# robin-karlsson0/pc-accumulation-lib

Measured on AMD Instinct MI355X. Metric: Mpoints/s projected+accumulated and BEV frames/s @256x256; 1/2/4/8 GPU, higher is better.
Workload: dtype f64; 1 GPU; KITTI-360 single forward cam, 120k pts/frame, 200 m horizon (~201 live frames, 5169634 stored pts), one 256x256x21 BEV per integrated frame; points_per_frame=120000, bev_px=256, view_m=80

## Files before the change

include/pca.h:

```cpp
#ifndef PCA_H
#define PCA_H

#include <stdint.h>

#ifdef __cplusplus
extern "C" {
#endif

#define PCA_VERSION 2

typedef struct pca_ctx pca_ctx;

typedef struct {
    double *x, *y, *z;
    float *intensity;
    uint32_t *rgbs;
    int32_t *inst;
    uint8_t *dyn;
    int64_t capacity;
    uint32_t *frame_box;
} pca_store;

#define PCA_STATUS_STORE_OVERFLOW 1u
#define PCA_STATUS_UV_OUT_OF_IMAGE 2u
// ... 121 lines not shown
    double *planes;
    uint16_t *planes_f16;
} pca_bev_job;
int pca_bev_generate_many(pca_ctx *ctx, const pca_store *store, const double *intensity64 ,
                          const int64_t *frame_off , const pca_bev_job *jobs, int n_jobs, int64_t max_points,
                          void *workspace , int64_t workspace_bytes, void *stream);

int pca_image_to_nchw_f32(pca_ctx *ctx, const uint8_t *rgb , int H, int W, const float mean[3], const float std[3],
                          float *out , void *stream);

int pca_bev_warp(pca_ctx *ctx, const uint16_t *planes_f16 , uint16_t *out_f16 , int n_planes, int px,
                 double a_1, double a_2, double b_1, double b_2, void *stream);

int pca_host_ego_to_grid(const double *full, int F, const double R[9], double dx, double dy, double view, int px,
                         double *rows, int32_t *start);

typedef struct pca_host_track pca_host_track;
typedef struct {
    const void *pts;
    const void *rgb;
    const void *sem;
    const void *sem_gt;
    int32_t n;
    uint32_t host_mask;
} pca_kitti_obs;
int pca_kitti_integrate(pca_ctx *ctx, const pca_kitti_obs *obs, const double P[12], int H, int W,
                        const uint64_t filter_mask[4], const pca_store *store, int64_t *frame_off , int slot,
                        int sample_mode, pca_host_track *track, const double *T_new_prev, double horizon, int64_t *evicted,
                        double *path_length, void *stream);
void pca_host_camera_cone(const double P[12], int H, int W, double cone[15]);
int pca_host_view_hull(int F, const double *then , const float *box , const double *cone ,
                       const double now[12], const pca_bev_params *prm, int *first, int *last);
int pca_bev_bin_range(pca_ctx *ctx, int slot_first, int slot_last_plus1);
int pca_bev_view_hint(pca_ctx *ctx, int slot0, int F, const double *then, const float *box, const double *cone, const double now[12],
                      const pca_bev_params *prm);
void pca_f32_box_decode(const uint32_t *rows , int n, float *box );

int pca_k1_defer(pca_ctx *ctx, int on);
int pca_k1_flush(pca_ctx *ctx);
int pca_kitti_generate_bev(pca_ctx *ctx, const pca_store *store, const int64_t *frame_off , int slot_begin,
                           int slot_split, int slot_end, int64_t max_points, const pca_bev_params *prm,
                           const double *pending_Ts, const int *pending_slot_ends, int n_pending, int write_back,
                           void *workspace , int64_t workspace_bytes, uint16_t *planes_f16 ,
                           void *host_planes , const pca_host_track *track, double *traj_rows,
                           int32_t *traj_start, int32_t *n_rows, void *stream);

typedef struct {
    const pca_kitti_obs *obs; const double *P; int32_t H, W; const uint64_t *filter_mask; const pca_store *store;
    int64_t *frame_off; int32_t slot, sample_mode; pca_host_track *track; const double *T_new_prev; double horizon;
    int64_t evicted; double path_length; void *stream;
} pca_kitti_integrate_args;
int pca_kitti_integrate_v(pca_ctx *ctx, pca_kitti_integrate_args *a);
typedef struct {
    const pca_store *store; const int64_t *frame_off; int32_t slot_begin, slot_split, slot_end, pad0; int64_t max_points;
    const pca_bev_params *prm; const double *pending_Ts; const int *pending_slot_ends; int32_t n_pending, write_back;
    void *workspace; int64_t workspace_bytes; uint16_t *planes_f16; void *host_planes; const pca_host_track *track;
    double *traj_rows; int32_t *traj_start; int32_t n_rows, pad1; void *stream;
    int32_t hint_slot0, hint_F; const double *hint_then; const float *hint_box; const double *hint_cone; const double *hint_now;
    int32_t hinted, pad2;
} pca_kitti_generate_bev_args;
int pca_kitti_generate_bev_v(pca_ctx *ctx, pca_kitti_generate_bev_args *a);

int pca_host_stage_h2d(int n, const void *const *src, void *const *pinned, void *const *dev, const int64_t *bytes,
                       void *stream);

int pca_host_d2h_async(pca_ctx *ctx, const void *dev, void *pinned, int64_t bytes, void *stream);
// ... 35 lines not shown
```

pc-accumulation-lib_amd/csrc/pca_bev.hip:

```cpp
#include "pca_bev_common.h"
#include "pca_k1_body.h"
#include <cstdlib>
#include <mutex>

#define KEY_INVALID 0xffffffffu
#define TS 8
#define TCELLS (TS * TS)
#define NFK (2 * TCELLS)
#ifndef AB_THREADS
#define AB_THREADS 1024
#endif
#define MAX_G 512
#ifndef BIN_RUNR
#define BIN_RUNR 4
#endif
#ifndef BIN_WPE
#define BIN_WPE 4
#endif
#ifndef BIN_UNR
#define BIN_UNR 4
#endif
#ifndef BIN_REG_P
#define BIN_REG_P 12
#endif
// ... 1365 lines not shown
            s_dyn[threadIdx.x] = w;
        }
        for (int t = threadIdx.x; t < n_hist; t += AB_THREADS) s_h[t] = 0;
        __syncthreads();
        const ViewConst vc = view_const(a);
        const uint32_t set = a.k1_slot >= a.slot_split ? 1u : 0u;
        const int lane = threadIdx.x & 63;
        uint32_t rkey[PPT];
#pragma unroll
        for (int r = 0; r < PPT; ++r) {
            const bool kept = (km[r] >> lane) & 1ull;
            rkey[r] = view_key_lean(vc, (double)p[r].x, (double)p[r].y, (double)p[r].z, kept, set);
            if (rkey[r] != KEY_INVALID) atomicAdd(&s_h[rkey[r] >> hs], 1u);
        }
        __syncthreads();
        bin_scan_tables(a, s_h, s_cur, s_wsum, split, (int)blockIdx.x);
        __syncthreads();
        const uint32_t seg = (uint32_t)blockIdx.x * K1_SEG;
#pragma unroll
        for (int r = 0; r < PPT; ++r) {
            if (rkey[r] == KEY_INVALID) continue;
            const uint32_t pos = seg + atomicAdd(&s_cur[rkey[r] >> hs], 1u);
            bin_store<false>(a, s_dyn, pos, rkey[r], packed[r], (double)p[r].z, 0.0, p[r].w);
        }
    }
};
static_assert(K1_SEG == 1024 * 4, "a K1 piece holds one 1024 x 4 tile");
__global__ __launch_bounds__(AB_THREADS) __attribute__((amdgpu_waves_per_eu(BIN_WPE, BIN_WPE))) void bev_tile_bin_k1(const BevArgs a, const K1Args k)
{
    if ((int)blockIdx.x < a.Gk) k1_body<AB_THREADS, 4, false, false, false>(k, BinK1Tail{a});
    else bev_tile_bin_body<false>(a);
}

template <bool I64>
__global__ __launch_bounds__(AB_THREADS) __attribute__((amdgpu_waves_per_eu(BIN_WPE, BIN_WPE))) void bev_tile_bin(const BevArgs a) { bev_tile_bin_body<I64>(a); }
#if C_THREADS == 512
#define C_OCC __attribute__((amdgpu_waves_per_eu(6, 6)))
#else
#define C_OCC
#endif
template <bool I64>
__global__ __launch_bounds__(C_THREADS) C_OCC void bev_tile_cells(const BevArgs a) { bev_tile_cells_body<I64>(a); }
template <bool I64, bool EXTRA, bool OWN>
__global__ __launch_bounds__(H_THREADS) void bev_tile_cells_heavy(const BevArgs a) { bev_tile_cells_heavy_body<I64, EXTRA, OWN>(a); }
#define PCA_BEV_MANY_MAX 48
__constant__ BevArgs g_bev_many[PCA_BEV_MANY_MAX];
template <bool I64>
__global__ __launch_bounds__(AB_THREADS) __attribute__((amdgpu_waves_per_eu(BIN_WPE, BIN_WPE))) void bev_tile_bin_many()
{
    const BevArgs &a = g_bev_many[blockIdx.y];
    if ((int)blockIdx.x < a.G) bev_tile_bin_body<I64>(a);
}
template <bool I64>
__global__ __launch_bounds__(C_THREADS) C_OCC void bev_tile_cells_many()
{
    bev_tile_cells_body<I64>(g_bev_many[blockIdx.y]);
}
template <bool I64>
__global__ __launch_bounds__(H_THREADS) void bev_tile_cells_heavy_many()
{
    bev_tile_cells_heavy_body<I64, false, false>(g_bev_many[blockIdx.y]);
}
template <bool I64>
__global__ __launch_bounds__(AB_THREADS) __attribute__((amdgpu_waves_per_eu(BIN_WPE, BIN_WPE))) void bev_tile_bin_band(const BevArgs a) { bev_tile_bin_body<I64, true>(a); }
template <bool I64>
__global__ __launch_bounds__(C_THREADS) C_OCC void bev_tile_cells_band(const BevArgs a) { bev_tile_cells_body<I64, true>(a); }
// ... 210 lines not shown
}

static size_t bev_decide_split(BevArgs &a, bool tuned)
{
    const int sp = tuned ? (int)PCA_ENV_ONCE("PCA_BEV_SPLIT", 1) : 0;
    a.split = (sp && a.heavy_launched && !a.intensity64 && (size_t)a.T * 16 <= 128 * 1024) ? (sp == 2 ? 2 : 1) : 0;
    return (size_t)a.T * 8 * (a.split ? 2 : 1);
}

static int bev_decide_k1_ride(pca_ctx *ctx, const BevArgs &a, bool tuned, size_t lds, hipStream_t s, K1Args *k1a, int *nt)
{
    *nt = 0;
    if (!ctx->k1_pend.valid) return 0;
    if (!tuned) return pca_k1_flush_pending(ctx);
    const int fk = (int)PCA_ENV_ONCE("PCA_FUSE_K1", 1);
    const pca_ctx::K1Pending &pd = ctx->k1_pend;
    bool owed_ok = true;
    for (int k = 0; k < a.n_pend; ++k) owed_ok = owed_ok && a.pend_slot_end[k] <= pd.slot;
    const bool fuse = fk && owed_ok && !a.intensity64 && pd.stream == s && pd.slot == a.slot_end - 1 && pd.slot >= a.slot_begin &&
                      pd.frame_off == a.frame_off && pd.store.x == a.st.x && lds <= K1_RIDE_LDS && pd.fr.n <= K1_RIDE * K1_SEG &&
                      pd.fr.n <= a.max_points && pca_k1_prepare_pending(ctx, k1a, nt, s) == 0 && *nt <= K1_RIDE;
    if (PCA_ENV_ONCE("PCA_FUSE_DBG", 0) && !fuse)
        fprintf(stderr, "bev: K1 of slot %d not taken along: switch %d owed_ok %d i64 %d stream %d slot %d (window %d..%d) frame_off %d store %d lds %zu n %d max_points %lld nt %d\n",
                pd.slot, fk, (int)owed_ok, a.intensity64 != nullptr, pd.stream == s, pd.slot == a.slot_end - 1, a.slot_begin, a.slot_end,
                pd.frame_off == a.frame_off, pd.store.x == a.st.x, lds, pd.fr.n, (long long)a.max_points, *nt);
    if (fuse) return 0;
    *nt = 0;
    return pca_k1_flush_pending(ctx);
}

struct BevBinRange { bool given; int first, end; };
static int bev_decide_bin_range(pca_ctx *ctx, BevArgs &a, bool tuned, const BevBinRange &r)
{
    if (!r.given || !PCA_ENV_ONCE("PCA_BEV_CULL", 1) || (a.n_pend > 0 && a.write_back)) return 0;
    const int f = r.first > a.slot_begin ? r.first : a.slot_begin, e = r.end < a.slot_end ? r.end : a.slot_end;
    a.bin_first = f; a.bin_end = e < f ? f : e;
    if (!tuned) return 0;
    const int64_t pts = PCA_ENV_ONCE("PCA_BEV_ONE_ROUND_PTS", 14500);
    a.span_hint = ctx->heavy_hint_dev + 1;
    a.span_hint_known = ctx->heavy_hint[1];
    return (pts > 0 && a.span_hint_known != 0 && (int64_t)a.span_hint_known * 1024 <= pts * ctx->n_cu && a.G > ctx->n_cu) ? ctx->n_cu : 0;
}

static void bev_size_level1(pca_ctx *ctx, BevArgs &a, int nt, int one_round)
{
    if (nt == 0) { if (one_round > 0) { a.G = one_round; bev_table_order(a); } return; }
    const pca_ctx::K1Pending &pd = ctx->k1_pend;
    const int cap = max_groups(), G0 = a.G;
    if (one_round) one_round -= nt;
    a.G = one_round > 0 ? one_round + nt : (G0 + nt <= cap || (cap - 2 * nt) * 4 < 3 * G0) ? G0 + nt : cap - nt;
    a.Gk = nt; bev_table_order(a); a.k1_slot = pd.slot; a.k1_n = pd.fr.n;
    a.max_points = a.max_points - pd.fr.n;
}

static int bev_launch_raster(pca_ctx *ctx, const BevKernelSet &ks, const BevArgs &a, const K1Args *k1, size_t lds, hipStream_t s)
{
    if (k1) {
        PCA_LAUNCH_SHM(ctx, PCA_K_BEV_BIN, bev_tile_bin_k1, dim3(a.G), dim3(AB_THREADS), lds, s, a, *k1);
        pca_k1_pending_launched(ctx, s);
    } else PCA_LAUNCH_SHM(ctx, PCA_K_BEV_BIN, ks.bin, dim3(a.G), dim3(AB_THREADS), lds, s, a);
    PCA_LAUNCH(ctx, PCA_K_BEV_CELLS, ks.cells, dim3(a.T), dim3(C_THREADS), s, a);
    if (!a.heavy_launched) return 0;
    const int heavy_grid = a.T < ctx->n_cu ? a.T : ctx->n_cu;
    const BevKernel heavy = ks.heavy[a.extra != nullptr][a.split != 0];
    if (!heavy) { ctx->err = "bev: no heavy kernel for a split banded raster"; return -1; }
    PCA_LAUNCH_SHM(ctx, PCA_K_BEV_CELLS_HEAVY, heavy, dim3(heavy_grid), dim3(H_THREADS), HEAVY_LDS_BYTES, s, a);
    return 0;
}

int pca_bev_generate_chain(pca_ctx *ctx, const pca_store *store, const double *intensity64, const int64_t *frame_off,
                           int slot_begin, int slot_split, int slot_end, int64_t max_points, const pca_bev_params *prm,
                           const double *pending_Ts, const int *pending_slot_ends, int n_pending, int write_back,
                           void *workspace, int64_t workspace_bytes, double *planes, uint16_t *planes_f16,
                           double *extra_planes, void *stream)
{
    if (!ctx) return -1;
    const BevBinRange bin_range = {ctx->bin_valid, ctx->bin_first, ctx->bin_end};
    ctx->bin_valid = false;
    if (max_points < 1) max_points = 1;
    hipStream_t s = (hipStream_t)stream;
    PCA_CHECK(ctx, hipSetDevice(ctx->device));
    BevArgs a;
    if (bev_prepare(ctx, store, intensity64, frame_off, slot_begin, slot_split, slot_end, max_points, prm, pending_Ts,
                    pending_slot_ends, n_pending, write_back, workspace, workspace_bytes, planes, planes_f16, extra_planes, a))
        return -1;
    if (bev_set_lds_attributes(ctx)) return -1;
    const bool tuned = a.band_rows == a.tx;
    const BevKernelSet &ks = g_bev_kernels[intensity64 != nullptr][!tuned];
    K1Args k1a;
    int nt = 0;
    bev_decide_heavy(ctx, a, tuned);
    const size_t lds = bev_decide_split(a, tuned);
    if (bev_decide_k1_ride(ctx, a, tuned, lds, s, &k1a, &nt)) return -1;
    const int one_round = bev_decide_bin_range(ctx, a, tuned, bin_range);
    bev_size_level1(ctx, a, nt, one_round);
    if (ctx->profiling == 2) pca_prof_begin(ctx, PCA_K_BEV_UNIT, s);
    for (int r0 = 0, rows = a.band_rows; r0 < a.tx; r0 += rows) {
        if (!tuned) {
            bev_set_band(a, r0);
            if (r0 > 0 && a.write_back) a.n_pend = 0;
        }
        if (bev_launch_raster(ctx, ks, a, nt ? &k1a : nullptr, lds, s)) return -1;
    }
    if (ctx->profiling == 2) pca_prof_end(ctx, s);
    PCA_CHECK(ctx, hipGetLastError());
    return 0;
}

int pca_bev_generate_many(pca_ctx *ctx, const pca_store *store, const double *intensity64, const int64_t *frame_off,
                          const pca_bev_job *jobs, int n_jobs, int64_t max_points, void *workspace,
                          int64_t workspace_bytes, void *stream)
{
    if (!ctx) return -1;
    if (pca_k1_flush_pending(ctx)) return -1;
    ctx->bin_valid = false;
    if (!jobs || n_jobs < 1) { ctx->err = "bev: bad job list"; return -1; }
    if (n_jobs > 65535) { ctx->err = "bev: at most 65535 rasters per call"; return -1; }
    if (max_points < 1) max_points = 1;
    hipStream_t s = (hipStream_t)stream;
    PCA_CHECK(ctx, hipSetDevice(ctx->device));
    const int px = jobs[0].prm.px;
    PX_CHECK(ctx, px);
    const BevLayout l = bev_layout(max_points, px);
    const int64_t per = l.total;
    if (workspace_bytes < per * n_jobs + 256) { ctx->err = "bev: workspace too small for this many rasters"; return -1; }
    const int rows = band_rows(px), n_bands = (tiles_x(px) + rows - 1) / rows;
    const BevKernelSet &ks = g_bev_kernels[intensity64 != nullptr][n_bands > 1];
    const int64_t up_bytes = (int64_t)sizeof(BevArgs) * n_jobs * n_bands;
    if (ctx->bevm_busy) { PCA_CHECK(ctx, hipEventSynchronize(ctx->bevm_ev)); ctx->bevm_busy = false; }
    if (up_bytes > ctx->bevm_cap) {
        if (ctx->bevm_pin) PCA_CHECK(ctx, hipHostFree(ctx->bevm_pin));
        ctx->bevm_pin = nullptr; ctx->bevm_cap = 0;
        PCA_CHECK(ctx, hipHostMalloc(&ctx->bevm_pin, (size_t)(2 * up_bytes), hipHostMallocMapped));
        ctx->bevm_cap = 2 * up_bytes;
    }
// ... 54 lines not shown
__device__ __forceinline__ int warp_src(double c1, double c2, int k, int n)
{
    const double kd = (double)k;
    double v = rint(c1 * kd + c2 * (kd * kd));
    v = v < 0.0 ? 0.0 : (v > (double)(n - 1) ? (double)(n - 1) : v);
    return (int)v;
}

__global__ __launch_bounds__(256) void bev_warp(const WarpArgs a)
{
    const int iw = blockIdx.x * 256 + threadIdx.x, jw = blockIdx.y;
    if (iw >= a.px) return;
    const int i = warp_src(a.a1, a.a2, iw, a.px), j = warp_src(a.b1, a.b2, jw, a.px);
    const size_t plane = (size_t)a.px * a.px;
    for (int n = 0; n < a.n_planes; ++n) a.out[n * plane + (size_t)jw * a.px + iw] = a.in[n * plane + (size_t)j * a.px + i];
}

int pca_bev_warp(pca_ctx *ctx, const uint16_t *planes_f16, uint16_t *out_f16, int n_planes, int px, double a_1, double a_2,
                 double b_1, double b_2, void *stream)
{
    if (!ctx) return -1;
    if (!planes_f16 || !out_f16 || planes_f16 == out_f16 || n_planes < 1 || px < 1 || px > 65535) { ctx->err = "warp: bad arguments"; return -1; }
    if (!(a_1 == a_1 && a_2 == a_2 && b_1 == b_1 && b_2 == b_2)) { ctx->err = "warp: NaN coefficient"; return -1; }
    hipStream_t s = (hipStream_t)stream;
    PCA_CHECK(ctx, hipSetDevice(ctx->device));
    WarpArgs a;
    a.in = planes_f16; a.out = out_f16; a.n_planes = n_planes; a.px = px;
    a.a1 = a_1; a.a2 = a_2; a.b1 = b_1; a.b2 = b_2;
    hipLaunchKernelGGL(bev_warp, dim3((px + 255) / 256, px), dim3(256), 0, s, a);
    PCA_CHECK(ctx, hipGetLastError());
    return 0;
}

int pca_debug_bev_stamps(unsigned long long *out)
{
    return (int)hipMemcpyFromSymbol(out, HIP_SYMBOL(g_dbg_stamps), sizeof(unsigned long long) * 8192);
}

}
```

pc-accumulation-lib_amd/csrc/pca_common.h:

```cpp
#pragma once
#include <hip/hip_runtime.h>
#include <stddef.h>
#include <stdint.h>
#include <stdlib.h>
#include <string>
#include <vector>

#include <hip/hip_fp16.h>
#include "../../include/pca.h"
#include "pca_wave.h"

#define PCA_WAVE 64

struct K1Frame {
    const float *pts;
    const uint8_t *rgb, *sem, *sem_gt;
    int32_t n;
    int32_t tile0;
    int32_t qpos0;
    int32_t f;
};

struct pca_ctx {
    int device = 0;
// ... 35 lines not shown
    int64_t k1_ws_cap[2] = {0, 0};
    K1Frame *k1_pin[2] = {nullptr, nullptr};
    int k1_pin_cap[2] = {0, 0};
    hipEvent_t k1_pin_ev[2] = {nullptr, nullptr};
    bool k1_pin_busy[2] = {false, false};
    int k1_pin_next = 0;
    unsigned long long *dbg = nullptr;
    int dbg_blocks = 0;
    int heavy_cooldown = 0;
    uint32_t *icp_cnt = nullptr;
    bool icp_cnt_dirty = true;
    double *icp_host = nullptr;
    double *icp_host_dev = nullptr;
    uint32_t icp_call = 0;
    struct K1Pending {
        bool valid = false;
        pca_kitti_frame fr;
        double P[12];
        int H = 0, W = 0;
        uint64_t filt[4] = {0, 0, 0, 0};
        pca_store store;
        int64_t *frame_off = nullptr;
        int slot = 0, sample_mode = 0;
        hipStream_t stream = nullptr;
        int stage_idx = -1;
    };
    bool k1_defer = false;
    K1Pending k1_pend;
    uint32_t *status_host = nullptr;
    uint32_t *heavy_hint = nullptr;
    uint32_t *heavy_hint_dev = nullptr;
    int bin_first = 0, bin_end = 0;
    bool bin_valid = false;
    struct Ev { hipEvent_t a, b; int kid; };
    int profiling = 0;
    std::vector<Ev> evs;
    std::vector<Ev> free_evs;
    double prof_ms[PCA_K_COUNT] = {0};
    int64_t prof_n[PCA_K_COUNT] = {0};
};

void pca_prof_begin(pca_ctx *ctx, int kid, hipStream_t s);
void pca_prof_end(pca_ctx *ctx, hipStream_t s);
#define PCA_LAUNCH_SHM(ctx, kid, kernel, grid, block, shm, stream, ...)        \
    do {                                                                        \
        if ((ctx)->profiling == 1) pca_prof_begin((ctx), (kid), (stream));      \
        hipLaunchKernelGGL(kernel, grid, block, shm, stream, __VA_ARGS__);      \
        if ((ctx)->profiling == 1) pca_prof_end((ctx), (stream));               \
    } while (0)
#define PCA_LAUNCH(ctx, kid, kernel, grid, block, stream, ...) \
    PCA_LAUNCH_SHM(ctx, kid, kernel, grid, block, 0, stream, __VA_ARGS__)

#define PCA_CHECK(ctx, expr)                                                                   \
    do {                                                                                       \
        hipError_t _e = (expr);                                                                \
        if (_e != hipSuccess) {                                                                \
            (ctx)->err = std::string(#expr) + ": " + hipGetErrorString(_e);                    \
            return -1;                                                                         \
        }                                                                                      \
    } while (0)

static inline int64_t pca_env_int(const char *name, int64_t dflt, int64_t lo = INT64_MIN, int64_t hi = INT64_MAX)
{
    const char *e = getenv(name);
    const int64_t v = e ? atoll(e) : dflt;
    return (v < lo || v > hi) ? dflt : v;
// ... 204 lines not shown
```

pc-accumulation-lib_amd/csrc/pca_session.hip:

```cpp
#include <vector>

#include "pca_common.h"

int pca_stage_copy(const void *const *src, void *const *dst, const int64_t *bytes, int n);

static inline int64_t up256(int64_t v) { return (v + 255) & ~255ll; }

extern "C" {

int pca_kitti_integrate(pca_ctx *ctx, const pca_kitti_obs *obs, const double P[12], int H, int W,
                        const uint64_t filter_mask[4], const pca_store *store, int64_t *frame_off, int slot, int sample_mode,
                        pca_host_track *track, const double *T_new_prev, double horizon, int64_t *evicted,
                        double *path_length, void *stream)
{
    if (!ctx) return -1;
    if (!obs || obs->n < 0 || !P || !filter_mask || !store || !frame_off) { ctx->err = "kitti_integrate: bad arguments"; return -1; }
    if (track && (!T_new_prev || !evicted || !path_length)) { ctx->err = "kitti_integrate: the pose track needs T_new_prev and its outputs"; return -1; }
    hipStream_t s = (hipStream_t)stream;
    PCA_CHECK(ctx, hipSetDevice(ctx->device));
    if (pca_k1_flush_pending(ctx)) return -1;
    const void *in[4] = {obs->pts, obs->rgb, obs->sem, obs->sem_gt};
    const int64_t size[4] = {16ll * obs->n, 3ll * H * W, 1ll * H * W, 1ll * obs->n};
    const void *dev[4] = {in[0], in[1], in[2], in[3]};
    int64_t off[4] = {0, 0, 0, 0}, total = 0;
// ... 42 lines not shown
                       obs->n <= (1 << 20);
    if (ctx->k1_defer && plain) {
        pca_ctx::K1Pending &pd = ctx->k1_pend;
        pd.fr = fr;
        for (int i = 0; i < 12; ++i) pd.P[i] = P[i];
        pd.H = H; pd.W = W;
        for (int i = 0; i < 4; ++i) pd.filt[i] = filter_mask[i];
        pd.store = *store; pd.frame_off = frame_off; pd.slot = slot; pd.sample_mode = sample_mode; pd.stream = s;
        pd.stage_idx = slot_st ? (int)(slot_st - ctx->stage) : -1;
        pd.valid = true;
    } else {
        const int rc = pca_kitti_project_sample_filter_ex(ctx, &fr, 1, P, H, W, filter_mask, store, frame_off, slot, sample_mode, stream);
        if (slot_st) {
            const hipError_t e = hipEventRecord(slot_st->done, s);
            if (e == hipSuccess) slot_st->busy = true;
            else {
                (void)hipStreamSynchronize(s);
                if (rc == 0) { ctx->err = std::string("kitti_integrate: hipEventRecord(stage done): ") + hipGetErrorString(e); return -1; }
            }
        }
        if (rc != 0) return rc;
    }
    if (track) *evicted = pca_host_track_step(track, T_new_prev, horizon, path_length);
    return 0;
}

int pca_kitti_generate_bev(pca_ctx *ctx, const pca_store *store, const int64_t *frame_off, int slot_begin, int slot_split,
                           int slot_end, int64_t max_points, const pca_bev_params *prm, const double *pending_Ts,
                           const int *pending_slot_ends, int n_pending, int write_back, void *workspace,
                           int64_t workspace_bytes, uint16_t *planes_f16, void *host_planes, const pca_host_track *track,
                           double *traj_rows, int32_t *traj_start, int32_t *n_rows, void *stream)
{
    if (!ctx) return -1;
    if (!prm || !planes_f16 || !track || !traj_rows || !traj_start || !n_rows) { ctx->err = "kitti_generate_bev: bad arguments"; return -1; }
    const int64_t F = pca_host_track_len(track);
    if (F != slot_end - slot_begin) { ctx->err = "kitti_generate_bev: the pose track and the window disagree about the number of frames"; return -1; }
    static thread_local std::vector<double> rel;
    rel.resize((size_t)(3 * (F > 0 ? F : 1)));
    const double *Hp = pca_host_track_poses(track);
    for (int64_t f = 0; f < F; ++f)
        for (int k = 0; k < 3; ++k) rel[(size_t)(3 * f + k)] = Hp[4 * f + k] - prm->origin[k];
    *n_rows = pca_host_ego_to_grid(rel.data(), (int)F, prm->R, prm->dx, prm->dy, prm->view, prm->px, traj_rows, traj_start);
    if (pca_bev_generate_chain(ctx, store, nullptr, frame_off, slot_begin, slot_split, slot_end, max_points, prm, pending_Ts,
                               pending_slot_ends, n_pending, write_back, workspace, workspace_bytes, nullptr, planes_f16,
                               nullptr, stream) != 0)
        return -1;
    if (!host_planes) return 0;
    return pca_host_d2h_async(ctx, planes_f16, host_planes, 21ll * prm->px * prm->px * 2, stream);
}

int pca_kitti_integrate_v(pca_ctx *ctx, pca_kitti_integrate_args *a)
{
    if (!ctx) return -1;
    if (!a) { ctx->err = "kitti_integrate_v: no argument block"; return -1; }
    return pca_kitti_integrate(ctx, a->obs, a->P, a->H, a->W, a->filter_mask, a->store, a->frame_off, a->slot, a->sample_mode,
                               a->track, a->T_new_prev, a->horizon, &a->evicted, &a->path_length, a->stream);
}

int pca_kitti_generate_bev_v(pca_ctx *ctx, pca_kitti_generate_bev_args *a)
{
    if (!ctx) return -1;
    if (!a) { ctx->err = "kitti_generate_bev_v: no argument block"; return -1; }
    a->hinted = 0;
    if (a->hint_F > 0 && !(a->n_pending > 0 && a->write_back)) {
        const int rc = pca_bev_view_hint(ctx, a->hint_slot0, a->hint_F, a->hint_then, a->hint_box, a->hint_cone, a->hint_now, a->prm);
        if (rc < 0) { ctx->err = "kitti_generate_bev_v: bad view hint"; return -1; }
        a->hinted = rc;
    }
    return pca_kitti_generate_bev(ctx, a->store, a->frame_off, a->slot_begin, a->slot_split, a->slot_end, a->max_points, a->prm,
                                  a->pending_Ts, a->pending_slot_ends, a->n_pending, a->write_back, a->workspace,
                                  a->workspace_bytes, a->planes_f16, a->host_planes, a->track, a->traj_rows, a->traj_start,
                                  &a->n_rows, a->stream);
}

}
```

pc-accumulation-lib_amd/pca_amd/_lib.py:

```python
import ctypes as C
import os
import threading

import numpy as np

_HERE = os.path.dirname(os.path.abspath(__file__))
LIB_PATH = os.path.join(_HERE, 'libpca_hip.so')

STATUS_STORE_OVERFLOW = 1
STATUS_UV_OUT_OF_IMAGE = 2
STATUS_NEGATIVE_INTENSITY = 4
STATUS_LOOKBACK_TIMEOUT = 8
SAMPLE_MODES = {'nearest': 0, 'bilinear': 1}

EXPORTS = ('pca_version', 'pca_ctx_create', 'pca_ctx_destroy', 'pca_last_error', 'pca_status', 'pca_status_peek', 'pca_status_mirror',
           'pca_kitti_project_sample_filter', 'pca_kitti_project_sample_filter_ex',
           'pca_nusc_sample_filter_transform', 'pca_nusc_sample_filter_transform_ex', 'pca_nusc_sample_filter_transform_batch', 'pca_sample_bilinear', 'pca_nusc_project_cams', 'pca_retransform', 'pca_retransform_batch_tail',
           'pca_mark_dynamic',
           'pca_bev_workspace_bytes', 'pca_bev_generate', 'pca_bev_generate_ex', 'pca_bev_generate_chain', 'pca_bev_generate_many', 'pca_bev_warp', 'pca_image_to_nchw_f32', 'pca_voxel_dedup_workspace_bytes', 'pca_voxel_dedup', 'pca_icp_workspace_bytes', 'pca_icp_register', 'pca_host_ego_to_grid',
           'pca_host_gemv4_probe', 'pca_host_gemv4_mode', 'pca_host_incr_probe', 'pca_host_incr_blocks', 'pca_host_track_create', 'pca_host_track_destroy', 'pca_host_track_len', 'pca_host_track_n_segments',
           'pca_host_track_poses', 'pca_host_track_segments', 'pca_host_track_set', 'pca_host_track_transform',
           'pca_host_track_append', 'pca_host_track_push_segment', 'pca_host_track_incr', 'pca_host_track_evict_beyond',
           'pca_host_track_step', 'pca_host_track_trigger', 'pca_host_stage_h2d', 'pca_host_d2h_async', 'pca_host_d2h_wait',
           'pca_kitti_integrate', 'pca_kitti_generate_bev', 'pca_k1_defer', 'pca_k1_flush', 'pca_host_camera_cone', 'pca_host_view_hull', 'pca_bev_bin_range', 'pca_bev_view_hint', 'pca_kitti_integrate_v', 'pca_kitti_generate_bev_v', 'pca_f32_box_decode',
           'pca_profile_enable', 'pca_profile_read')

KERNEL_IDS = ('kitti_project_sample_filter', 'nusc_sample_filter_transform', 'nusc_project_cams', 'retransform',
              'mark_dynamic', 'bev_bin', 'bev_scan', 'bev_scatter', 'bev_cells', 'bev_cells_heavy', 'voxel_dedup', 'bev_unit', 'icp')
BEV_EXTRA_PLANES = ('elevation_max', 'elevation_mean', 'intensity_mean')


class PcaStore(C.Structure):
    _fields_ = [('x', C.c_void_p), ('y', C.c_void_p), ('z', C.c_void_p), ('intensity', C.c_void_p),
                ('rgbs', C.c_void_p), ('inst', C.c_void_p), ('dyn', C.c_void_p), ('capacity', C.c_int64),
                ('frame_box', C.c_void_p)]


class PcaKittiIntegrateArgs(C.Structure):
    _fields_ = [('obs', C.c_void_p), ('P', C.c_void_p), ('H', C.c_int32), ('W', C.c_int32), ('filter_mask', C.c_void_p),
                ('store', C.c_void_p), ('frame_off', C.c_void_p), ('slot', C.c_int32), ('sample_mode', C.c_int32),
                ('track', C.c_void_p), ('T_new_prev', C.c_void_p), ('horizon', C.c_double), ('evicted', C.c_int64),
                ('path_length', C.c_double), ('stream', C.c_void_p)]


class PcaKittiGenerateBevArgs(C.Structure):
    _fields_ = [('store', C.c_void_p), ('frame_off', C.c_void_p), ('slot_begin', C.c_int32), ('slot_split', C.c_int32),
                ('slot_end', C.c_int32), ('pad0', C.c_int32), ('max_points', C.c_int64), ('prm', C.c_void_p),
                ('pending_Ts', C.c_void_p), ('pending_slot_ends', C.c_void_p), ('n_pending', C.c_int32), ('write_back', C.c_int32),
                ('workspace', C.c_void_p), ('workspace_bytes', C.c_int64), ('planes_f16', C.c_void_p), ('host_planes', C.c_void_p),
                ('track', C.c_void_p), ('traj_rows', C.c_void_p), ('traj_start', C.c_void_p), ('n_rows', C.c_int32),
                ('pad1', C.c_int32), ('stream', C.c_void_p), ('hint_slot0', C.c_int32), ('hint_F', C.c_int32),
                ('hint_then', C.c_void_p), ('hint_box', C.c_void_p), ('hint_cone', C.c_void_p), ('hint_now', C.c_void_p),
                ('hinted', C.c_int32), ('pad2', C.c_int32)]


class PcaKittiObs(C.Structure):
    _fields_ = [('pts', C.c_void_p), ('rgb', C.c_void_p), ('sem', C.c_void_p), ('sem_gt', C.c_void_p),
# ... 120 lines not shown
    lib.pca_host_track_create.argtypes = [C.POINTER(vp), vp]
    lib.pca_host_track_destroy.argtypes = [vp]
    lib.pca_host_track_destroy.restype = None
    for name in ('pca_host_track_len', 'pca_host_track_n_segments'):
        getattr(lib, name).argtypes = [vp]
        getattr(lib, name).restype = i64
    for name in ('pca_host_track_poses', 'pca_host_track_segments'):
        getattr(lib, name).argtypes = [vp]
        getattr(lib, name).restype = vp
    lib.pca_host_track_set.argtypes = [vp, vp, i64, vp, i64]
    lib.pca_host_track_transform.argtypes = [vp, vp]
    lib.pca_host_track_append.argtypes = [vp, vp]
    lib.pca_host_track_push_segment.argtypes = [vp, dp]
    lib.pca_host_track_incr.argtypes = [vp, vp]
    lib.pca_host_track_evict_beyond.argtypes = [vp, C.c_double, C.c_double]
    lib.pca_host_track_evict_beyond.restype = i64
    lib.pca_host_track_step.argtypes = [vp, vp, C.c_double, dp]
    lib.pca_host_track_step.restype = i64
    lib.pca_host_track_trigger.argtypes = [vp, C.c_double, i64, C.c_double]
    lib.pca_host_track_trigger.restype = i64
    lib.pca_host_stage_h2d.argtypes = [i32, vp, vp, vp, vp, vp]
    lib.pca_host_d2h_async.argtypes = [vp, vp, vp, i64, vp]
    lib.pca_host_d2h_wait.argtypes = [vp, i32]
    lib.pca_kitti_integrate.argtypes = [vp, C.POINTER(PcaKittiObs), C.POINTER(C.c_double), i32, i32, C.POINTER(C.c_uint64),
                                        C.POINTER(PcaStore), vp, i32, i32, vp, vp, C.c_double, C.POINTER(C.c_int64),
                                        C.POINTER(C.c_double), vp]
    lib.pca_kitti_generate_bev.argtypes = [vp, C.POINTER(PcaStore), vp, i32, i32, i32, i64, C.POINTER(PcaBevParams), vp, vp,
                                           i32, i32, vp, i64, vp, vp, vp, vp, vp, C.POINTER(C.c_int32), vp]
    lib.pca_host_camera_cone.argtypes = [vp, i32, i32, vp]
    lib.pca_host_camera_cone.restype = None
    lib.pca_host_view_hull.argtypes = [i32, vp, vp, vp, vp, vp, C.POINTER(C.c_int), C.POINTER(C.c_int)]
    lib.pca_bev_bin_range.argtypes = [vp, i32, i32]
    lib.pca_bev_view_hint.argtypes = [vp, i32, i32, vp, vp, vp, vp, vp]
    lib.pca_f32_box_decode.argtypes = [vp, i32, vp]
    lib.pca_f32_box_decode.restype = None
    lib.pca_kitti_integrate_v.argtypes = [vp, vp]
    lib.pca_kitti_generate_bev_v.argtypes = [vp, vp]
    lib.pca_k1_defer.argtypes = [vp, i32]
    lib.pca_k1_flush.argtypes = [vp]
    lib.pca_profile_enable.argtypes = [vp, i32]
    lib.pca_profile_read.argtypes = [vp, i32, C.POINTER(C.c_double), C.POINTER(C.c_int64)]
    _lib = lib
    return lib


class Context:

    _by_device = {}
    _raw_stream = None
    _tls = threading.local()

    def __init__(self, device_index):
        import torch
        if not torch.cuda.is_available():
            raise RuntimeError('pca_amd needs an AMD GPU (torch.cuda.is_available() is False); '
                               'there is no CPU fallback')
        self.lib = load()
        self.device_index = int(device_index)
        h = C.c_void_p()
        if self.lib.pca_ctx_create(self.device_index, C.byref(h)) != 0:
            raise RuntimeError('pca_ctx_create failed')
        self.h = h
        self._mirror = (C.c_uint32 * 8).from_address(self.lib.pca_status_mirror(h))
        self._mirror_q = (C.c_uint64 * 4).from_address(C.addressof(self._mirror))

    @classmethod
# ... 4 lines not shown
                               'there is no CPU fallback')
        idx = torch.cuda.current_device() if device is None else torch.device(device).index or 0
        lane = getattr(cls._tls, 'lane', None)
        if lane is not None and lane.device_index == idx:
            return lane
        if idx not in cls._by_device:
            cls._by_device[idx] = Context(idx)
        return cls._by_device[idx]

    def destroy(self):
        if self.h is not None:
            self.lib.pca_ctx_destroy(self.h)
            self.h = None

    def stream(self):
        return C.c_void_p(self.stream_int())

    def stream_int(self):
        raw = self._raw_stream
        if raw is None:
            import torch
            raw = getattr(torch._C, '_cuda_getCurrentRawStream', None)
            if raw is None:
                return torch.cuda.current_stream(self.device_index).cuda_stream
            self._raw_stream = raw
        return raw(self.device_index)

    def check(self, rc):
        if rc != 0:
            raise RuntimeError('pca: ' + self.lib.pca_last_error(self.h).decode())

    def profile(self, on):
        self.check(self.lib.pca_profile_enable(self.h, int(on)))

    def profile_read(self):
        out = {}
        for k, name in enumerate(KERNEL_IDS):
            ms, n = C.c_double(0), C.c_int64(0)
            self.check(self.lib.pca_profile_read(self.h, k, C.byref(ms), C.byref(n)))
            out[name] = (ms.value, n.value)
        return out

    def peek_status(self):
        q = self._mirror_q
        if not (q[0] | q[1] | q[2] | q[3]):
            return 0
        m = self._mirror
        return sum(1 << b for b in range(8) if m[b])

    def check_status(self):
        st = self.status()
        if not st:
            return
        said = [(STATUS_UV_OUT_OF_IMAGE, AssertionError, 'pts_uv must be all inside image'),
                (STATUS_STORE_OVERFLOW, RuntimeError, 'pca: device point store overflow (points were dropped)'),
                (STATUS_LOOKBACK_TIMEOUT, RuntimeError,
                 'pca: a compaction workgroup timed out waiting for its predecessor (output invalid)'),
                (STATUS_NEGATIVE_INTENSITY, ValueError, 'pca: negative lidar intensity on the f32 path (pass intensity64 to bev())')]
        hit = [(exc, msg) for bit, exc, msg in said if st & bit]
        rest = st & ~(STATUS_UV_OUT_OF_IMAGE | STATUS_STORE_OVERFLOW | STATUS_LOOKBACK_TIMEOUT | STATUS_NEGATIVE_INTENSITY)
        if rest:
            hit.append((RuntimeError, 'pca: unknown device status bits 0x%x' % rest))
        raise hit[0][0]('; '.join(msg for _, msg in hit))

    def poll_status(self):
        if self.peek_status():
# ... 39 lines not shown
```

pc-accumulation-lib_amd/pca_amd/device_store.py:

```python
import ctypes as C
import os

import numpy as np
import torch

from . import _lib
from ._lib import PcaBevParams, PcaKittiFrame, PcaStore

CULL = os.environ.get('PCA_BEV_CULL', '1') != '0'


class DeviceStore:
    CHAIN_MAX = 4
    CHAIN_K = int(os.environ.get('PCA_BEV_CHAIN', '4'))

    def __init__(self, capacity=1 << 24, max_frames=4096, device=None, intensity_div255=False):
        self.ctx = _lib.Context.get(device)
        self.device = torch.device('cuda', self.ctx.device_index)
        self.intensity_div255 = bool(intensity_div255)
        self.max_frames = int(max_frames)
        self._alloc(int(capacity))
        self.frame_off = torch.zeros(self.max_frames + 1, dtype=torch.int64, device=self.device)
        self._moved = np.eye(4)
        self.cull = CULL
# ... 81 lines not shown
            n = self.tail - self.head
            if n > 0:
                if self._box_pin is None or self._box_pin.shape[0] < self.frame_box.shape[0]:
                    self._box_pin = torch.empty(tuple(self.frame_box.shape), dtype=torch.int32, pin_memory=True)
                self._box_pin[:n].copy_(self.frame_box[self.head:self.tail], non_blocking=True)
                ev = torch.cuda.Event()
                ev.record()
                self._box_copy = (ev, self.head, n)
                self._since_box = 0

    def _poll_boxes(self):
        if self._box_copy is None or not self._box_copy[0].query():
            return
        _, first, n = self._box_copy
        self._box_copy = None
        rows = self._box_pin[:n].numpy()
        dec = np.empty((n, 6), dtype=np.float32)
        self.ctx.lib.pca_f32_box_decode(rows.ctypes.data, n, dec.ctypes.data)
        known = dec[:, 0] <= dec[:, 1]
        tgt = self._box[first:first + n]
        tgt[known] = dec[known]

    def view_hint_into(self, args, first_frame, last_frame):
        n = last_frame - first_frame
        if not self.cull or n < 4:
            return 0
        a = self.head + first_frame
        args.hint_slot0 = a
        args.hint_then, args.hint_box = self._then_addr + 96 * a, self._box_addr + 24 * a
        args.hint_cone = self._cone[2] if (self._cone is not None and self._n_nocone == 0) else None
        args.hint_now = self._moved.ctypes.data
        return n

    def view_hint(self, prm, first_frame, last_frame, write_back):
        n = last_frame - first_frame
        if not self.cull or write_back or n < 4:
            return 0
        a = self.head + first_frame
        cone = self._cone[2] if (self._cone is not None and self._n_nocone == 0) else None
        return self._count_hint(self.ctx.lib.pca_bev_view_hint(self.ctx.h, a, n, self._then_addr + 96 * a, self._box_addr + 24 * a, cone,
                                              self._moved.ctypes.data, C.addressof(prm)))

    def _count_hint(self, r):
        self.hints_taken += 1 if r > 0 else 0
        return r

    def c_store(self):
        if self._cstore is None:
            self._cstore = PcaStore(self.x.data_ptr(), self.y.data_ptr(), self.z.data_ptr(), self.intensity.data_ptr(),
                                    self.rgbs.data_ptr(), self.inst.data_ptr(), self.dyn.data_ptr(), self.capacity,
                                    self.frame_box.data_ptr())
        return self._cstore

    @property
    def n_frames(self):
        return self.tail - self.head

    def set_defer_k1(self, on):
        self.ctx.check(self.ctx.lib.pca_k1_defer(self.ctx.h, 1 if on else 0))
        self.ctx.k1_defer = bool(on)
        if not on:
            self._k1_noted = None

    def flush_k1(self):
        if self._k1_noted is not None:
            self.ctx.check(self.ctx.lib.pca_k1_flush(self.ctx.h))
            self._k1_noted = None

    def __del__(self):
# ... 263 lines not shown
        ctx = self.ctx
        ctx.check(ctx.lib.pca_mark_dynamic(ctx.h, C.byref(st), self.frame_off.data_ptr(), slots, insts, len(pairs),
                                           ctx.stream()))

    def voxel_dedup(self, voxel_size):
        if self.n_frames == 0:
            return
        self.flush_pending()
        ctx, lib = self.ctx, self.ctx.lib
        max_points = self.max_window_points()
        need = lib.pca_voxel_dedup_workspace_bytes(max_points, self.n_frames)
        if self._dedup_ws is None or self._dedup_ws.numel() < need:
            self._dedup_ws = torch.empty(int(need) + 256, dtype=torch.uint8, device=self.device)
        st = self.c_store()
        ctx.check(lib.pca_voxel_dedup(ctx.h, C.byref(st), self.frame_off.data_ptr(), self.head, self.tail,
                                      float(voxel_size), max_points, self._dedup_ws.data_ptr(),
                                      self._dedup_ws.numel(), ctx.stream()))

    def bev(self, split_frame, prm, want_f64=False, intensity64=None, first_frame=0, last_frame=None, out16=None,
            extra=None):
        ctx, lib = self.ctx, self.ctx.lib
        last_frame = self.n_frames if last_frame is None else last_frame
        px = int(prm.px)
        max_points = self.bev_workspace(px)
        if out16 is not None:
            assert out16.dtype == torch.float16 and out16.is_contiguous() and tuple(out16.shape) == (21, px, px)
        p16 = out16 if out16 is not None else torch.empty((21, px, px), dtype=torch.float16, device=self.device)
        p64 = torch.empty((21, px, px), dtype=torch.float64, device=self.device) if want_f64 else None
        st = self.c_store()
        n_pend, pend_T, pend_ends, write_back = self.bev_pending(first_frame, last_frame)
        if extra is not None:
            assert extra.dtype == torch.float64 and extra.is_contiguous() \
                and tuple(extra.shape) == (3, len(_lib.BEV_EXTRA_PLANES), px, px)
        self.view_hint(prm, first_frame, last_frame, n_pend > 0 and write_back)
        ctx.check(lib.pca_bev_generate_chain(ctx.h, C.byref(st), None if intensity64 is None else intensity64.data_ptr(),
                                             self.frame_off.data_ptr(), self.head + first_frame, self.head + split_frame,
                                             self.head + last_frame, max_points, C.byref(prm), pend_T, pend_ends, n_pend,
                                             write_back, self._ws.data_ptr(), self._ws.numel(),
                                             None if p64 is None else p64.data_ptr(), p16.data_ptr(),
                                             None if extra is None else extra.data_ptr(), ctx.stream()))
        self.bev_done(write_back)
        return p16, p64

    def bev_workspace(self, px):
        max_points = self.max_window_points()
        if self._ws is None or max_points > self._ws_points or px != self._ws_px:
            self._ws_points, self._ws_px = int(max_points * 1.25) + 1, px
            need = self.ctx.lib.pca_bev_workspace_bytes(self._ws_points, px)
            if self._ws is None or self._ws.numel() < need:
                self._ws = torch.empty(int(need) + 256, dtype=torch.uint8, device=self.device)
        return max_points

    def bev_pending(self, first_frame, last_frame):
        if not self._pending:
            return 0, None, None, 1
        if first_frame != 0 or self._pending[-1][1] > self.head + last_frame:
            self.flush_pending()
            return 0, None, None, 1
        n_pend = 0
        for T, e in self._pending:
            if e > self.head:
                self._pend_T_np[16 * n_pend:16 * n_pend + 16] = T
                self._pend_ends[n_pend] = int(e)
                n_pend += 1
        if n_pend == 0:
            return 0, None, None, 0
        return n_pend, self._pend_T, self._pend_ends, (1 if n_pend >= self.CHAIN_K else 0)
# ... 112 lines not shown
```

Before: 1442 Mpoints/s.

## Allow view-culled binning during write-back by streaming owed transforms for skipped frames

```diff
diff --git a/include/pca.h b/include/pca.h
--- a/include/pca.h
+++ b/include/pca.h
@@ -177,6 +177,7 @@
 int pca_host_view_hull(int F, const double *then , const float *box , const double *cone ,
                        const double now[12], const pca_bev_params *prm, int *first, int *last);
 int pca_bev_bin_range(pca_ctx *ctx, int slot_first, int slot_last_plus1);
+int pca_bev_write_back_range_stats(pca_ctx *ctx, int64_t *calls, int64_t *points);
 int pca_bev_view_hint(pca_ctx *ctx, int slot0, int F, const double *then, const float *box, const double *cone, const double now[12],
                       const pca_bev_params *prm);
 void pca_f32_box_decode(const uint32_t *rows , int n, float *box );
diff --git a/pc-accumulation-lib_amd/csrc/pca_bev.hip b/pc-accumulation-lib_amd/csrc/pca_bev.hip
--- a/pc-accumulation-lib_amd/csrc/pca_bev.hip
+++ b/pc-accumulation-lib_amd/csrc/pca_bev.hip
@@ -1421,6 +1421,64 @@
     else bev_tile_bin_body<false>(a);
 }
 
+#define SO_THREADS 256
+struct BevStreamArgs {
+    double *x, *y, *z;
+    const int64_t *frame_off;
+    int slot_begin, bin_first, bin_end, n_pend;
+    int pend_slot_end[PCA_BEV_MAX_CHAIN];
+    Mat34 pend_T[PCA_BEV_MAX_CHAIN];
+    unsigned long long *points;
+};
+__device__ __forceinline__ void stream_owed_point(const BevStreamArgs &a, const PendHi &pend_hi, int64_t p, double &X, double &Y, double &Z)
+{
+#pragma unroll 1
+    for (int k = 0; k < a.n_pend; ++k) {
+        const int64_t hi = k == 0 ? pend_hi.v[0] : k == 1 ? pend_hi.v[1] : k == 2 ? pend_hi.v[2] : pend_hi.v[3];
+        if (p < hi) {
+            const Mat34 &T = a.pend_T[k];
+            const double nx = row4(T.m + 0, X, Y, Z), ny = row4(T.m + 4, X, Y, Z), nz = row4(T.m + 8, X, Y, Z);
+            X = nx; Y = ny; Z = nz;
+        }
+    }
+}
+__global__ __launch_bounds__(SO_THREADS) void bev_stream_owed(const BevStreamArgs a)
+{
+    const int e_new = a.pend_slot_end[a.n_pend - 1];
+    const int64_t base = a.frame_off[a.slot_begin];
+    PendHi pend_hi;
+#pragma unroll
+    for (int k = 0; k < PCA_BEV_MAX_CHAIN; ++k)
+        pend_hi.v[k] = (k < a.n_pend && a.pend_slot_end[k] > a.slot_begin) ? a.frame_off[a.pend_slot_end[k]] : base;
+    const int a_end = a.bin_first < e_new ? a.bin_first : e_new, b_end = a.bin_end > e_new ? a.bin_end : e_new;
+    const int64_t lo[2] = {base, a.frame_off[a.bin_end]};
+    const int64_t hi[2] = {a_end > a.slot_begin ? a.frame_off[a_end] : base, a.frame_off[b_end]};
+    const int64_t gtid = (int64_t)blockIdx.x * SO_THREADS + threadIdx.x, gsz = (int64_t)gridDim.x * SO_THREADS;
+    if (gtid == 0) *a.points += (unsigned long long)((hi[0] - lo[0]) + (hi[1] - lo[1]));
+    int64_t lo2[2], n2[2];
+#pragma unroll
+    for (int s = 0; s < 2; ++s) {
+        lo2[s] = (lo[s] + 1) & ~1ll;
+        const int64_t hi2 = hi[s] & ~1ll;
+        n2[s] = hi2 > lo2[s] ? (hi2 - lo2[s]) / 2 : 0;
+        const int64_t single = (gtid == 2 * s + 1) ? ((lo[s] < lo2[s] && lo[s] < hi[s]) ? lo[s] : -1)
+                             : (gtid == 2 * s + 2) ? ((hi2 < hi[s] && hi2 >= lo2[s]) ? hi2 : -1) : -1;
+        if (single >= 0) {
+            double X = a.x[single], Y = a.y[single], Z = a.z[single];
+            stream_owed_point(a, pend_hi, single, X, Y, Z);
+            a.x[single] = X; a.y[single] = Y; a.z[single] = Z;
+        }
+    }
+    double2 *X2 = reinterpret_cast<double2 *>(a.x), *Y2 = reinterpret_cast<double2 *>(a.y), *Z2 = reinterpret_cast<double2 *>(a.z);
+    for (int64_t i = gtid; i < n2[0] + n2[1]; i += gsz) {
+        const int64_t q = i < n2[0] ? lo2[0] / 2 + i : lo2[1] / 2 + (i - n2[0]);
+        double2 vx = X2[q], vy = Y2[q], vz = Z2[q];
+        stream_owed_point(a, pend_hi, 2 * q, vx.x, vy.x, vz.x);
+        stream_owed_point(a, pend_hi, 2 * q + 1, vx.y, vy.y, vz.y);
+        X2[q] = vx; Y2[q] = vy; Z2[q] = vz;
+    }
+}
+
 template <bool I64>
 __global__ __launch_bounds__(AB_THREADS) __attribute__((amdgpu_waves_per_eu(BIN_WPE, BIN_WPE))) void bev_tile_bin(const BevArgs a) { bev_tile_bin_body<I64>(a); }
 #if C_THREADS == 512
@@ -1697,14 +1755,31 @@
 struct BevBinRange { bool given; int first, end; };
 static int bev_decide_bin_range(pca_ctx *ctx, BevArgs &a, bool tuned, const BevBinRange &r)
 {
-    if (!r.given || !PCA_ENV_ONCE("PCA_BEV_CULL", 1) || (a.n_pend > 0 && a.write_back)) return 0;
-    const int f = r.first > a.slot_begin ? r.first : a.slot_begin, e = r.end < a.slot_end ? r.end : a.slot_end;
+    if (!r.given || !PCA_ENV_ONCE("PCA_BEV_CULL", 1)) return 0;
+    if (a.n_pend > 0 && a.write_back && (!tuned || a.intensity64 || !pca_env_int("PCA_BEV_WB_CULL", 1))) return 0;
+    const int f0 = r.first > a.slot_begin ? r.first : a.slot_begin, f = f0 < a.slot_end ? f0 : a.slot_end;
+    const int e = r.end < a.slot_end ? r.end : a.slot_end;
     a.bin_first = f; a.bin_end = e < f ? f : e;
     if (!tuned) return 0;
     const int64_t pts = PCA_ENV_ONCE("PCA_BEV_ONE_ROUND_PTS", 14500);
     a.span_hint = ctx->heavy_hint_dev + 1;
     a.span_hint_known = ctx->heavy_hint[1];
     return (pts > 0 && a.span_hint_known != 0 && (int64_t)a.span_hint_known * 1024 <= pts * ctx->n_cu && a.G > ctx->n_cu) ? ctx->n_cu : 0;
+}
+
+static bool bev_decide_stream_owed(pca_ctx *ctx, const BevArgs &a, BevStreamArgs *sa)
+{
+    if (!(a.n_pend > 0 && a.write_back) || (a.bin_first == a.slot_begin && a.bin_end == a.slot_end)) return false;
+    ++ctx->wb_range_calls;
+    sa->x = a.st.x; sa->y = a.st.y; sa->z = a.st.z;
+    sa->frame_off = a.frame_off;
+    sa->slot_begin = a.slot_begin; sa->bin_first = a.bin_first;
+    sa->bin_end = (a.Gk && a.k1_slot < a.bin_end) ? a.k1_slot : a.bin_end;
+    sa->n_pend = a.n_pend;
+    for (int k = 0; k < PCA_BEV_MAX_CHAIN; ++k) { sa->pend_slot_end[k] = a.pend_slot_end[k]; sa->pend_T[k] = a.pend_T[k]; }
+    sa->points = reinterpret_cast<unsigned long long *>(ctx->heavy_hint_dev + 2);
+    const int e_new = a.pend_slot_end[a.n_pend - 1];
+    return (sa->bin_first > a.slot_begin && e_new > a.slot_begin) || e_new > sa->bin_end;
 }
 
 static void bev_size_level1(pca_ctx *ctx, BevArgs &a, int nt, int one_round)
@@ -1718,12 +1793,18 @@
     a.max_points = a.max_points - pd.fr.n;
 }
 
-static int bev_launch_raster(pca_ctx *ctx, const BevKernelSet &ks, const BevArgs &a, const K1Args *k1, size_t lds, hipStream_t s)
-{
-    if (k1) {
-        PCA_LAUNCH_SHM(ctx, PCA_K_BEV_BIN, bev_tile_bin_k1, dim3(a.G), dim3(AB_THREADS), lds, s, a, *k1);
-        pca_k1_pending_launched(ctx, s);
-    } else PCA_LAUNCH_SHM(ctx, PCA_K_BEV_BIN, ks.bin, dim3(a.G), dim3(AB_THREADS), lds, s, a);
+static int bev_launch_raster(pca_ctx *ctx, const BevKernelSet &ks, const BevArgs &a, const K1Args *k1, const BevStreamArgs *sa, size_t lds,
+                             hipStream_t s)
+{
+    if (ctx->profiling == 1) pca_prof_begin(ctx, PCA_K_BEV_BIN, s);
+    if (sa) {
+        const int64_t blocks = (a.max_points + 4 * SO_THREADS - 1) / (4 * SO_THREADS);
+        hipLaunchKernelGGL(bev_stream_owed, dim3((unsigned)(blocks < 1 ? 1 : blocks > 2048 ? 2048 : blocks)), dim3(SO_THREADS), 0, s, *sa);
+    }
+    if (k1) hipLaunchKernelGGL(bev_tile_bin_k1, dim3(a.G), dim3(AB_THREADS), lds, s, a, *k1);
+    else hipLaunchKernelGGL(ks.bin, dim3(a.G), dim3(AB_THREADS), lds, s, a);
+    if (ctx->profiling == 1) pca_prof_end(ctx, s);
+    if (k1) pca_k1_pending_launched(ctx, s);
     PCA_LAUNCH(ctx, PCA_K_BEV_CELLS, ks.cells, dim3(a.T), dim3(C_THREADS), s, a);
     if (!a.heavy_launched) return 0;
     const int heavy_grid = a.T < ctx->n_cu ? a.T : ctx->n_cu;
@@ -1759,13 +1840,15 @@
     if (bev_decide_k1_ride(ctx, a, tuned, lds, s, &k1a, &nt)) return -1;
     const int one_round = bev_decide_bin_range(ctx, a, tuned, bin_range);
     bev_size_level1(ctx, a, nt, one_round);
+    BevStreamArgs sa;
+    const bool stream_owed = bev_decide_stream_owed(ctx, a, &sa);
     if (ctx->profiling == 2) pca_prof_begin(ctx, PCA_K_BEV_UNIT, s);
     for (int r0 = 0, rows = a.band_rows; r0 < a.tx; r0 += rows) {
         if (!tuned) {
             bev_set_band(a, r0);
             if (r0 > 0 && a.write_back) a.n_pend = 0;
         }
-        if (bev_launch_raster(ctx, ks, a, nt ? &k1a : nullptr, lds, s)) return -1;
+        if (bev_launch_raster(ctx, ks, a, nt ? &k1a : nullptr, stream_owed ? &sa : nullptr, lds, s)) return -1;
     }
     if (ctx->profiling == 2) pca_prof_end(ctx, s);
     PCA_CHECK(ctx, hipGetLastError());
@@ -1886,6 +1969,14 @@
     return 0;
 }
 
+int pca_bev_write_back_range_stats(pca_ctx *ctx, int64_t *calls, int64_t *points)
+{
+    if (!ctx) return -1;
+    if (calls) *calls = ctx->wb_range_calls;
+    if (points) *points = (int64_t)*reinterpret_cast<volatile unsigned long long *>(ctx->heavy_hint + 2);
+    return 0;
+}
+
 int pca_debug_bev_stamps(unsigned long long *out)
 {
     return (int)hipMemcpyFromSymbol(out, HIP_SYMBOL(g_dbg_stamps), sizeof(unsigned long long) * 8192);
diff --git a/pc-accumulation-lib_amd/csrc/pca_common.h b/pc-accumulation-lib_amd/csrc/pca_common.h
--- a/pc-accumulation-lib_amd/csrc/pca_common.h
+++ b/pc-accumulation-lib_amd/csrc/pca_common.h
@@ -91,6 +91,7 @@
     uint32_t *heavy_hint_dev = nullptr;
     int bin_first = 0, bin_end = 0;
     bool bin_valid = false;
+    int64_t wb_range_calls = 0;
     struct Ev { hipEvent_t a, b; int kid; };
     int profiling = 0;
     std::vector<Ev> evs;
diff --git a/pc-accumulation-lib_amd/csrc/pca_session.hip b/pc-accumulation-lib_amd/csrc/pca_session.hip
--- a/pc-accumulation-lib_amd/csrc/pca_session.hip
+++ b/pc-accumulation-lib_amd/csrc/pca_session.hip
@@ -98,9 +98,9 @@
                            double *traj_rows, int32_t *traj_start, int32_t *n_rows, void *stream)
 {
     if (!ctx) return -1;
-    if (!prm || !planes_f16 || !track || !traj_rows || !traj_start || !n_rows) { ctx->err = "kitti_generate_bev: bad arguments"; return -1; }
+    if (!prm || !planes_f16 || !track || !traj_rows || !traj_start || !n_rows) { ctx->bin_valid = false; ctx->err = "kitti_generate_bev: bad arguments"; return -1; }
     const int64_t F = pca_host_track_len(track);
-    if (F != slot_end - slot_begin) { ctx->err = "kitti_generate_bev: the pose track and the window disagree about the number of frames"; return -1; }
+    if (F != slot_end - slot_begin) { ctx->bin_valid = false; ctx->err = "kitti_generate_bev: the pose track and the window disagree about the number of frames"; return -1; }
     static thread_local std::vector<double> rel;
     rel.resize((size_t)(3 * (F > 0 ? F : 1)));
     const double *Hp = pca_host_track_poses(track);
@@ -128,7 +128,7 @@
     if (!ctx) return -1;
     if (!a) { ctx->err = "kitti_generate_bev_v: no argument block"; return -1; }
     a->hinted = 0;
-    if (a->hint_F > 0 && !(a->n_pending > 0 && a->write_back)) {
+    if (a->hint_F > 0) {
         const int rc = pca_bev_view_hint(ctx, a->hint_slot0, a->hint_F, a->hint_then, a->hint_box, a->hint_cone, a->hint_now, a->prm);
         if (rc < 0) { ctx->err = "kitti_generate_bev_v: bad view hint"; return -1; }
         a->hinted = rc;
diff --git a/pc-accumulation-lib_amd/pca_amd/_lib.py b/pc-accumulation-lib_amd/pca_amd/_lib.py
--- a/pc-accumulation-lib_amd/pca_amd/_lib.py
+++ b/pc-accumulation-lib_amd/pca_amd/_lib.py
@@ -22,7 +22,7 @@
            'pca_host_track_poses', 'pca_host_track_segments', 'pca_host_track_set', 'pca_host_track_transform',
            'pca_host_track_append', 'pca_host_track_push_segment', 'pca_host_track_incr', 'pca_host_track_evict_beyond',
            'pca_host_track_step', 'pca_host_track_trigger', 'pca_host_stage_h2d', 'pca_host_d2h_async', 'pca_host_d2h_wait',
-           'pca_kitti_integrate', 'pca_kitti_generate_bev', 'pca_k1_defer', 'pca_k1_flush', 'pca_host_camera_cone', 'pca_host_view_hull', 'pca_bev_bin_range', 'pca_bev_view_hint', 'pca_kitti_integrate_v', 'pca_kitti_generate_bev_v', 'pca_f32_box_decode',
+           'pca_kitti_integrate', 'pca_kitti_generate_bev', 'pca_k1_defer', 'pca_k1_flush', 'pca_host_camera_cone', 'pca_host_view_hull', 'pca_bev_bin_range', 'pca_bev_write_back_range_stats', 'pca_bev_view_hint', 'pca_kitti_integrate_v', 'pca_kitti_generate_bev_v', 'pca_f32_box_decode',
            'pca_profile_enable', 'pca_profile_read')
 
 KERNEL_IDS = ('kitti_project_sample_filter', 'nusc_sample_filter_transform', 'nusc_project_cams', 'retransform',
@@ -209,6 +209,7 @@
     lib.pca_host_view_hull.argtypes = [i32, vp, vp, vp, vp, vp, C.POINTER(C.c_int), C.POINTER(C.c_int)]
     lib.pca_bev_bin_range.argtypes = [vp, i32, i32]
     lib.pca_bev_view_hint.argtypes = [vp, i32, i32, vp, vp, vp, vp, vp]
+    lib.pca_bev_write_back_range_stats.argtypes = [vp, C.POINTER(C.c_int64), C.POINTER(C.c_int64)]
     lib.pca_f32_box_decode.argtypes = [vp, i32, vp]
     lib.pca_f32_box_decode.restype = None
     lib.pca_kitti_integrate_v.argtypes = [vp, vp]
@@ -279,6 +280,13 @@
 
     def profile(self, on):
         self.check(self.lib.pca_profile_enable(self.h, int(on)))
+
+    def write_back_range_stats(self):
+        import torch
+        torch.cuda.synchronize(self.device_index)
+        calls, points = C.c_int64(0), C.c_int64(0)
+        self.check(self.lib.pca_bev_write_back_range_stats(self.h, C.byref(calls), C.byref(points)))
+        return calls.value, points.value
 
     def profile_read(self):
         out = {}
diff --git a/pc-accumulation-lib_amd/pca_amd/device_store.py b/pc-accumulation-lib_amd/pca_amd/device_store.py
--- a/pc-accumulation-lib_amd/pca_amd/device_store.py
+++ b/pc-accumulation-lib_amd/pca_amd/device_store.py
@@ -137,9 +137,9 @@
         args.hint_now = self._moved.ctypes.data
         return n
 
-    def view_hint(self, prm, first_frame, last_frame, write_back):
+    def view_hint(self, prm, first_frame, last_frame):
         n = last_frame - first_frame
-        if not self.cull or write_back or n < 4:
+        if not self.cull or n < 4:
             return 0
         a = self.head + first_frame
         cone = self._cone[2] if (self._cone is not None and self._n_nocone == 0) else None
@@ -469,7 +469,7 @@
         if extra is not None:
             assert extra.dtype == torch.float64 and extra.is_contiguous() \
                 and tuple(extra.shape) == (3, len(_lib.BEV_EXTRA_PLANES), px, px)
-        self.view_hint(prm, first_frame, last_frame, n_pend > 0 and write_back)
+        self.view_hint(prm, first_frame, last_frame)
         ctx.check(lib.pca_bev_generate_chain(ctx.h, C.byref(st), None if intensity64 is None else intensity64.data_ptr(),
                                              self.frame_off.data_ptr(), self.head + first_frame, self.head + split_frame,
                                              self.head + last_frame, max_points, C.byref(prm), pend_T, pend_ends, n_pend,
```

Result: no change. 1434 Mpoints/s (-0.5%).
